# Anima-Lab/MaskDiT

Measured on AMD Instinct MI355X. Metric: training img/sec MaskDiT-XL/2 256 mask=0.5 bs=1024, higher is better.
Workload: dtype bf16; 1 GPU; DiT-XL/2 ImageNet256-latent [32x32x4], mask_ratio=0.5, mae_loss_coef=0.1, sample(moments)+class-dropout+fwd+bwd+grad-allreduce+AdamW+EMA, random-init (de-zeroed) weights; global_batch=1024, per_gpu_batch=1024, micro_batch=1024, accum=1, parallelism=dp1

## Files before the change

maskdit_amd/csrc/attention.hip:

```cpp
#include "common.h"
#include <type_traits>
#include "../../include/maskdit_hip.h"

template <int HD>
struct AttnCfg {
  static constexpr int HDK = (HD + 31) / 32 * 32;
  static constexpr int HDN = (HD + 15) / 16 * 16;
  static constexpr int KSTEPS = HDK / 32;
  static constexpr int NFRAG = HDN / 16;
  static constexpr int CH = HD / 8;
  static constexpr int PITCH_CH = (HDK / 8) | 1;
  static constexpr int PITCH = PITCH_CH * 16;
  static constexpr int TILE_BYTES = 64 * PITCH;
};

template <int HD> struct AttnRow {
  static constexpr int NFRAG = AttnCfg<HD>::NFRAG;
  static constexpr int NP = (NFRAG / 2 < HD / 32) ? NFRAG / 2 : HD / 32;
  static constexpr int NT = NFRAG - 2 * NP;
  uint4 pr[NP > 0 ? NP : 1];
  uint2 tl[NT > 0 ? NT : 1];
};
__device__ __forceinline__ unsigned attn_pack2(float a, float b) {
  bf16x2 t;
// ... 666 lines not shown
    for (int qi = 0; qi < QF; ++qi) {
#pragma unroll
      for (int f = 0; f < C::NFRAG; ++f) o[qi][f] = (f32x4){0.f, 0.f, 0.f, 0.f};
      m_run[qi] = -1e30f;
      l_run[qi] = 0.f;
    }
#pragma unroll 1
    for (int kb = 0; kb < L; kb += KB) {
      f32x4 s[QF][KB / 16];
#pragma unroll
      for (int f = 0; f < KB / 16; ++f) {
#pragma unroll
        for (int qi = 0; qi < QF; ++qi) s[qi][f] = (f32x4){0.f, 0.f, 0.f, 0.f};
#pragma unroll
        for (int ks = 0; ks < C::KSTEPS; ++ks) {
          const bf16x8 kfr = sp_frag_rows<HD, L>(Ks, kb + 16 * f + i16, ks, g);
#pragma unroll
          for (int qi = 0; qi < QF; ++qi) s[qi][f] = mfma16(kfr, qf[qi][ks], s[qi][f]);
        }
      }
      bf16x8 pf[QF][KB / 32];
      if (kb + KB > Lv) {
#pragma unroll
        for (int qi = 0; qi < QF; ++qi)
#pragma unroll
          for (int f = 0; f < KB / 16; ++f)
#pragma unroll
            for (int r = 0; r < 4; ++r) s[qi][f][r] = (kb + 16 * f + 4 * g + r < Lv) ? s[qi][f][r] : -1e30f;
      }
#pragma unroll
      for (int qi = 0; qi < QF; ++qi) {
        float mx = -1e30f;
#pragma unroll
        for (int f = 0; f < KB / 16; ++f)
#pragma unroll
          for (int r = 0; r < 4; ++r) mx = fmaxf(mx, s[qi][f][r]);
        mx = group_max(mx);
        const float m_new = fmaxf(m_run[qi], mx * scale_log2e);
        const float alpha = fast_exp2(m_run[qi] - m_new);
        float psum = 0.f;
#pragma unroll
        for (int f = 0; f < KB / 16; ++f)
#pragma unroll
          for (int r = 0; r < 4; ++r) {
            const float pv = fast_exp2(__builtin_fmaf(s[qi][f][r], scale_log2e, -m_new));
            s[qi][f][r] = pv;
            psum += pv;
          }
        l_run[qi] = l_run[qi] * alpha + psum;
        m_run[qi] = m_new;
#pragma unroll
        for (int f = 0; f < C::NFRAG; ++f)
#pragma unroll
          for (int r = 0; r < 4; ++r) o[qi][f][r] *= alpha;
#pragma unroll
        for (int ks = 0; ks < KB / 32; ++ks) pf[qi][ks] = pack_pair(s[qi][2 * ks], s[qi][2 * ks + 1]);
      }
#pragma unroll
      for (int ks = 0; ks < KB / 32; ++ks)
#pragma unroll
        for (int f = 0; f < C::NFRAG; ++f) {
          const bf16x8 vfr = sp_frag_cols<HD, L>(Vs, kb + 32 * ks, f, i16, g);
#pragma unroll
          for (int qi = 0; qi < QF; ++qi) o[qi][f] = mfma16(vfr, pf[qi][ks], o[qi][f]);
        }
    }
#pragma unroll
    for (int qi = 0; qi < QF; ++qi) {
      const int q = wave * 16 * KF + 16 * (qp + qi) + i16;
      const float l_tot = group_sum(l_run[qi]);
      const float inv = 1.f / l_tot;
      bf16* orow = out + ((long)b * L + q) * D + h * HD;
      AttnRow<HD> orw;
      attn_pack_row<HD>(orw, o[qi], inv);
      attn_store_row<HD>(orow, g, orw);
      if (g == 0) lse[((long)b * H + h) * L + q] = m_run[qi] + log2f(l_tot);
    }
  }
}

__device__ __forceinline__ void sp_item_coords(int item, int B, int H, int& b, int& h) {
  const int full = (B >> 3) << 3;
  int sid;
  if (item < full * H) {
    const int xcd = item & 7, k = item >> 3;
    const int grp = k / H;
    sid = (grp * 8 + xcd) * H + (k - grp * H);
  } else {
    sid = item;
  }
  b = sid / H;
  h = sid - b * H;
}

#define SP_LDS_BARRIER()                                 \
  {                                                      \
    asm volatile("s_waitcnt lgkmcnt(0)" ::: "memory");   \
    __builtin_amdgcn_s_barrier();                        \
    asm volatile("" ::: "memory");                       \
  }
template <int HD, int KF, int OCC>
__global__ __launch_bounds__(512, OCC) void attn_bwd_sp_kernel(const bf16* __restrict__ qkv, const bf16* __restrict__ out,
                                                              const bf16* __restrict__ dout, const float* __restrict__ lse,
                                                              float* __restrict__ delta, bf16* __restrict__ dqkv, int H,
                                                              float scale, float scale_log2e, int Lv, int B, int dbg) {
  using C = SpCfg<HD>;
  constexpr int L = 128 * KF;
  constexpr int TILE = L * C::PITCH;
  __shared__ __attribute__((aligned(16))) char smem[4 * TILE + 2 * L * 4 + 64];
  char* Qs = smem;
  char* Ks = smem + TILE;
  char* Vs = smem + 2 * TILE;
  char* dOs = smem + 3 * TILE;
  float* lse_s = (float*)(smem + 4 * TILE);
  float* del_s = lse_s + L;
  const int tid = threadIdx.x, lane = tid & 63, wave = tid >> 6;
  const int i16 = lane & 15, g = lane >> 4;
  const int D = H * HD;
  const long ld = 3L * D;
  const int nitems = B * H;

  SpRegs<HD, L> r0, r1, r2, r3;
  bf16x8 of[KF][C::KSTEPS], dof[KF][C::KSTEPS];
  float lse_r = 0.f;
  auto fetch = [&](int item) {
    int b, h;
    sp_item_coords(item, B, H, b, h);
    const bf16* base = qkv + (long)b * L * ld + h * HD;
    const bf16* dobase = dout + (long)b * L * D + h * HD;
    const bf16* obase = out + (long)b * L * D + h * HD;
    sp_load_nb<HD, L>(r0, base, ld, tid);
    sp_load_nb<HD, L>(r1, base + D, ld, tid);
    sp_load_nb<HD, L>(r2, base + 2 * D, ld, tid);
    sp_load_nb<HD, L>(r3, dobase, D, tid);
    lse_r = lse[((long)b * H + h) * L + (tid & (L - 1))];
#pragma unroll
    for (int qi = 0; qi < KF; ++qi) {
      const int q = wave * 16 * KF + 16 * qi + i16;
#pragma unroll
      for (int s = 0; s < C::KSTEPS; ++s) {
        const int d = min(32 * s + 8 * g, HD - 8);
        of[qi][s] = *(const bf16x8*)(obase + (long)q * D + d);
        dof[qi][s] = *(const bf16x8*)(dobase + (long)q * D + d);
      }
    }
  };

  auto stage = [&](int it) {
    int b, h;
    sp_item_coords(it, B, H, b, h);
    const long bh = (long)b * H + h;
    sp_store<HD, L>(r0, Qs, tid);
    sp_store<HD, L>(r1, Ks, tid);
    sp_store<HD, L>(r2, Vs, tid);
    sp_store<HD, L>(r3, dOs, tid);
    if (tid < L) lse_s[tid] = lse_r;
#pragma unroll
    for (int qi = 0; qi < KF; ++qi) {
      const int q = wave * 16 * KF + 16 * qi + i16;
      float dl = 0.f;
#pragma unroll
      for (int s = 0; s < C::KSTEPS; ++s) {
        float part = 0.f;
#pragma unroll
        for (int e = 0; e < 8; ++e) part += bf2f(dof[qi][s][e]) * bf2f(of[qi][s][e]);
        dl += (32 * s + 8 * g < HD) ? part : 0.f;
      }
      dl = group_sum(dl);
      if (g == 0) {
        del_s[q] = dl * scale;
        delta[bh * L + q] = dl;
      }
    }
  };

  int item = blockIdx.x;
  if (item >= nitems) return;
  fetch(item);
  stage(item);
  for (;;) {
    int b, h;
    sp_item_coords(item, B, H, b, h);
    SP_LDS_BARRIER()
    const bool has_next = OCC == 2 && item + (int)gridDim.x < nitems;
    if (has_next && !MDT_EXP(dbg & 2)) fetch(item + gridDim.x);
    __builtin_amdgcn_sched_barrier(0);

#pragma unroll 1
    for (int ki = 0; ki < (MDT_EXP(dbg & 4) ? 0 : KF); ++ki) {
      const int k0 = wave * 16 * KF + 16 * ki;
      bf16x8 kf[C::KSTEPS], vf[C::KSTEPS];
#pragma unroll
      for (int ks = 0; ks < C::KSTEPS; ++ks) {
        kf[ks] = sp_frag_rows<HD, L>(Ks, k0 + i16, ks, g);
        vf[ks] = sp_frag_rows<HD, L>(Vs, k0 + i16, ks, g);
      }
      f32x4 dk[C::NFRAG], dv[C::NFRAG];
#pragma unroll
      for (int f = 0; f < C::NFRAG; ++f) {
        dk[f] = (f32x4){0.f, 0.f, 0.f, 0.f};
        dv[f] = (f32x4){0.f, 0.f, 0.f, 0.f};
      }
      const bool key_ok = (k0 + i16) < Lv;
#pragma unroll 1
      for (int qb = 0; qb < L; qb += 64) {
        f32x4 pm[4], ds[4];
#pragma unroll
        for (int f = 0; f < 4; ++f) {
          f32x4 s = (f32x4){0.f, 0.f, 0.f, 0.f}, dp = (f32x4){0.f, 0.f, 0.f, 0.f};
#pragma unroll
          for (int ks = 0; ks < C::KSTEPS; ++ks) {
            s = mfma16(sp_frag_rows<HD, L>(Qs, qb + 16 * f + i16, ks, g), kf[ks], s);
            dp = mfma16(sp_frag_rows<HD, L>(dOs, qb + 16 * f + i16, ks, g), vf[ks], dp);
          }
          const f32x4 ls = *(const f32x4*)(lse_s + qb + 16 * f + 4 * g);
          const f32x4 dl = *(const f32x4*)(del_s + qb + 16 * f + 4 * g);
#pragma unroll
          for (int r = 0; r < 4; ++r) {
            const float pv = fast_exp2(__builtin_fmaf(s[r], scale_log2e, -ls[r]));
            pm[f][r] = pv;
            ds[f][r] = pv * __builtin_fmaf(dp[r], scale, -dl[r]);
          }
        }
#pragma unroll
        for (int ks = 0; ks < 2; ++ks) {
          const bf16x8 pf = pack_pair(pm[2 * ks], pm[2 * ks + 1]);
          const bf16x8 dsf = pack_pair(ds[2 * ks], ds[2 * ks + 1]);
#pragma unroll
          for (int f = 0; f < C::NFRAG; ++f) {
            dv[f] = mfma16(sp_frag_cols<HD, L>(dOs, qb + 32 * ks, f, i16, g), pf, dv[f]);
            dk[f] = mfma16(sp_frag_cols<HD, L>(Qs, qb + 32 * ks, f, i16, g), dsf, dk[f]);
          }
        }
      }
      bf16* drow = dqkv + ((long)b * L + k0 + i16) * ld + h * HD;
      AttnRow<HD> krw, vrw;
      if (!key_ok) {
#pragma unroll
        for (int f = 0; f < C::NFRAG; ++f) dk[f] = dv[f] = (f32x4){0.f, 0.f, 0.f, 0.f};
      }
      attn_pack_row<HD>(krw, dk);
      attn_pack_row<HD>(vrw, dv);
      if (!MDT_EXP(dbg & 1)) {
        attn_store_row<HD>(drow + D, g, krw);
        attn_store_row<HD>(drow + 2 * D, g, vrw);
      }
    }

#pragma unroll 1
    for (int qi = 0; qi < (MDT_EXP(dbg & 8) ? 0 : KF); ++qi) {
      const int q = wave * 16 * KF + 16 * qi + i16;
      bf16x8 qf[C::KSTEPS], dqo[C::KSTEPS];
#pragma unroll
      for (int ks = 0; ks < C::KSTEPS; ++ks) {
        qf[ks] = sp_frag_rows<HD, L>(Qs, q, ks, g);
        dqo[ks] = sp_frag_rows<HD, L>(dOs, q, ks, g);
      }
      const float my_lse = lse_s[q], dl = del_s[q];
      f32x4 dq[C::NFRAG];
#pragma unroll
      for (int f = 0; f < C::NFRAG; ++f) dq[f] = (f32x4){0.f, 0.f, 0.f, 0.f};
#pragma unroll 1
      for (int kb = 0; kb < L; kb += 64) {
        f32x4 ds[4];
#pragma unroll
        for (int f = 0; f < 4; ++f) {
          f32x4 s = (f32x4){0.f, 0.f, 0.f, 0.f}, dp = (f32x4){0.f, 0.f, 0.f, 0.f};
#pragma unroll
          for (int ks = 0; ks < C::KSTEPS; ++ks) {
            s = mfma16(sp_frag_rows<HD, L>(Ks, kb + 16 * f + i16, ks, g), qf[ks], s);
            dp = mfma16(sp_frag_rows<HD, L>(Vs, kb + 16 * f + i16, ks, g), dqo[ks], dp);
          }
#pragma unroll
          for (int r = 0; r < 4; ++r) {
            const float pv = fast_exp2(__builtin_fmaf(s[r], scale_log2e, -my_lse));
            ds[f][r] = pv * __builtin_fmaf(dp[r], scale, -dl);
          }
        }
        if (kb + 64 > Lv) {
#pragma unroll
          for (int f = 0; f < 4; ++f)
#pragma unroll
            for (int r = 0; r < 4; ++r) ds[f][r] = (kb + 16 * f + 4 * g + r < Lv) ? ds[f][r] : 0.f;
        }
#pragma unroll
        for (int ks = 0; ks < 2; ++ks) {
          const bf16x8 dsf = pack_pair(ds[2 * ks], ds[2 * ks + 1]);
#pragma unroll
          for (int f = 0; f < C::NFRAG; ++f) dq[f] = mfma16(sp_frag_cols<HD, L>(Ks, kb + 32 * ks, f, i16, g), dsf, dq[f]);
        }
      }
      bf16* drow = dqkv + ((long)b * L + q) * ld + h * HD;
      AttnRow<HD> qrw;
      attn_pack_row<HD>(qrw, dq);
      if (!MDT_EXP(dbg & 1)) attn_store_row<HD>(drow, g, qrw);
    }
    if (!has_next) break;
    SP_LDS_BARRIER()
    item += gridDim.x;
    stage(item);
  }
}

template <int HD>
__device__ __forceinline__ void attn_bwd_item_math(const char* Qs, const char* Ks, const char* Vs, const char* dOs,
                                                   const float* lse_s, const float* del_s, bf16* dbase, long ld, int D,
                                                   int wave, int i16, int g, int Lv, float scale, float scale_log2e,
                                                   AttnRow<HD>& q_cur, const AttnRow<HD>& q_prev) {
  using C = SpCfg<HD>;
  constexpr int L = 128;
  AttnRow<HD> k_keep, v_keep;
  {
    const int k0 = wave * 16;
    bf16x8 kf[C::KSTEPS], vf[C::KSTEPS];
#pragma unroll
    for (int ks = 0; ks < C::KSTEPS; ++ks) {
      kf[ks] = sp_frag_rows<HD, L>(Ks, k0 + i16, ks, g);
      vf[ks] = sp_frag_rows<HD, L>(Vs, k0 + i16, ks, g);
    }
    f32x4 dk[C::NFRAG], dv[C::NFRAG];
#pragma unroll
    for (int f = 0; f < C::NFRAG; ++f) {
      dk[f] = (f32x4){0.f, 0.f, 0.f, 0.f};
      dv[f] = (f32x4){0.f, 0.f, 0.f, 0.f};
    }
    const bool key_ok = (k0 + i16) < Lv;
#pragma unroll 1
    for (int qb = 0; qb < L; qb += 64) {
      f32x4 pm[4], ds[4];
#pragma unroll
      for (int f = 0; f < 4; ++f) {
        f32x4 s = (f32x4){0.f, 0.f, 0.f, 0.f}, dp = (f32x4){0.f, 0.f, 0.f, 0.f};
#pragma unroll
        for (int ks = 0; ks < C::KSTEPS; ++ks) {
          s = mfma16(sp_frag_rows<HD, L>(Qs, qb + 16 * f + i16, ks, g), kf[ks], s);
          dp = mfma16(sp_frag_rows<HD, L>(dOs, qb + 16 * f + i16, ks, g), vf[ks], dp);
        }
        const f32x4 ls = *(const f32x4*)(lse_s + qb + 16 * f + 4 * g);
        const f32x4 dl = *(const f32x4*)(del_s + qb + 16 * f + 4 * g);
#pragma unroll
        for (int r = 0; r < 4; ++r) {
          const float pv = fast_exp2(__builtin_fmaf(s[r], scale_log2e, -ls[r]));
          pm[f][r] = pv;
          ds[f][r] = pv * __builtin_fmaf(dp[r], scale, -dl[r]);
        }
      }
#pragma unroll
      for (int ks = 0; ks < 2; ++ks) {
        const bf16x8 pf = pack_pair(pm[2 * ks], pm[2 * ks + 1]);
        const bf16x8 dsf = pack_pair(ds[2 * ks], ds[2 * ks + 1]);
#pragma unroll
        for (int f = 0; f < C::NFRAG; ++f) {
          dv[f] = mfma16(sp_frag_cols<HD, L>(dOs, qb + 32 * ks, f, i16, g), pf, dv[f]);
          dk[f] = mfma16(sp_frag_cols<HD, L>(Qs, qb + 32 * ks, f, i16, g), dsf, dk[f]);
        }
      }
    }
    bf16* drow = dbase + (long)(k0 + i16) * ld;
    if (!key_ok) {
#pragma unroll
      for (int f = 0; f < C::NFRAG; ++f) dk[f] = dv[f] = (f32x4){0.f, 0.f, 0.f, 0.f};
    }
    attn_pack_row<HD>(k_keep, dk);
    attn_pack_row<HD>(v_keep, dv);
    attn_store_row<HD>(drow + D, g, k_keep);
    attn_store_row<HD>(drow + 2 * D, g, v_keep);
    attn_keep_alive<HD>(q_prev);
  }
  {
    const int q = wave * 16 + i16;
    bf16x8 qf[C::KSTEPS], dqo[C::KSTEPS];
#pragma unroll
    for (int ks = 0; ks < C::KSTEPS; ++ks) {
      qf[ks] = sp_frag_rows<HD, L>(Qs, q, ks, g);
      dqo[ks] = sp_frag_rows<HD, L>(dOs, q, ks, g);
    }
    const float my_lse = lse_s[q], dl = del_s[q];
    f32x4 dq[C::NFRAG];
#pragma unroll
    for (int f = 0; f < C::NFRAG; ++f) dq[f] = (f32x4){0.f, 0.f, 0.f, 0.f};
#pragma unroll 1
    for (int kb = 0; kb < L; kb += 64) {
      f32x4 ds[4];
#pragma unroll
      for (int f = 0; f < 4; ++f) {
        f32x4 s = (f32x4){0.f, 0.f, 0.f, 0.f}, dp = (f32x4){0.f, 0.f, 0.f, 0.f};
#pragma unroll
        for (int ks = 0; ks < C::KSTEPS; ++ks) {
          s = mfma16(sp_frag_rows<HD, L>(Ks, kb + 16 * f + i16, ks, g), qf[ks], s);
          dp = mfma16(sp_frag_rows<HD, L>(Vs, kb + 16 * f + i16, ks, g), dqo[ks], dp);
        }
#pragma unroll
        for (int r = 0; r < 4; ++r) {
          const float pv = fast_exp2(__builtin_fmaf(s[r], scale_log2e, -my_lse));
          ds[f][r] = pv * __builtin_fmaf(dp[r], scale, -dl);
        }
      }
      if (kb + 64 > Lv) {
#pragma unroll
        for (int f = 0; f < 4; ++f)
#pragma unroll
          for (int r = 0; r < 4; ++r) ds[f][r] = (kb + 16 * f + 4 * g + r < Lv) ? ds[f][r] : 0.f;
      }
#pragma unroll
      for (int ks = 0; ks < 2; ++ks) {
        const bf16x8 dsf = pack_pair(ds[2 * ks], ds[2 * ks + 1]);
#pragma unroll
        for (int f = 0; f < C::NFRAG; ++f) dq[f] = mfma16(sp_frag_cols<HD, L>(Ks, kb + 32 * ks, f, i16, g), dsf, dq[f]);
      }
    }
    bf16* drow = dbase + (long)q * ld;
    attn_pack_row<HD>(q_cur, dq);
    attn_store_row<HD>(drow, g, q_cur);
    attn_keep_alive<HD>(k_keep);
    attn_keep_alive<HD>(v_keep);
  }
}

template <int HD>
__global__ __launch_bounds__(512, 2) void attn_bwd_dma_kernel(const bf16* __restrict__ qkv, const bf16* __restrict__ out,
                                                               const bf16* __restrict__ dout, const float* __restrict__ lse,
                                                               float* __restrict__ delta, bf16* __restrict__ dqkv, int H,
                                                               float scale, float scale_log2e, int Lv, int B) {
  using C = SpCfg<HD>;
  static_assert(C::PITCH == HD * 2, "tile rows must be contiguous in LDS (odd chunk count)");
  constexpr int L = 128;
  constexpr int TILE = L * C::PITCH;
  constexpr int HALF_CH = L * C::CH / 2;
  static_assert(HALF_CH % 64 == 0, "a wave moves whole 1-KiB pieces");
  constexpr int NDMA = HALF_CH / 64;
  constexpr int NSTORE = 1 + 3 * (AttnRow<HD>::NP + AttnRow<HD>::NT);
  __shared__ __attribute__((aligned(16))) char buf0[4 * TILE];
  __shared__ __attribute__((aligned(16))) char buf1[4 * TILE];
  __shared__ float lse_s0[L], lse_s1[L], del_s[L];
  const int tid = threadIdx.x, lane = tid & 63;
  const int wave = __builtin_amdgcn_readfirstlane(tid >> 6);
  const int i16 = lane & 15, g = lane >> 4;
  const int D = H * HD;
  const long ld = 3L * D;
  const int nitems = B * H;

  static_assert(NDMA == 9, "nine 1-KiB pieces per wave");
  const int tw = wave >> 1, hw = wave & 1;
  const long row_bytes = (tw < 3 ? ld : (long)D) * 2;
  unsigned doff[NDMA];
  int lds_main, lds_tail;
  if constexpr (sp_split<HD, L>) {
#pragma unroll
    for (int j = 0; j < 8; ++j) {
      const int r = 64 * hw + 8 * j + (lane >> 3), c = (lane & 7) ^ (lane >> 3);
      doff[j] = (unsigned)(r * row_bytes + c * 16);
    }
    doff[8] = (unsigned)((64 * hw + lane) * row_bytes + 128);
    lds_main = tw * TILE + hw * 8192;
    lds_tail = tw * TILE + L * 128 + hw * 1024;
  } else {
#pragma unroll
    for (int j = 0; j < NDMA; ++j) {
      const int idx = hw * HALF_CH + 64 * j + lane;
      const int r = idx / C::CH, c = idx - r * C::CH;
      doff[j] = (unsigned)(r * row_bytes + c * 16);
    }
    lds_main = tw * TILE + hw * HALF_CH * 16;
    lds_tail = lds_main + 8192;
  }
  auto item_src = [&](int item) -> const char* {
    int b, h;
    sp_item_coords(item, B, H, b, h);
    return tw < 3 ? (const char*)(qkv + (long)b * L * ld + h * HD + tw * D) : (const char*)(dout + (long)b * L * D + h * HD);
  };

  float lse_r = 0.f;
  bf16x8 of0[C::KSTEPS], of1[C::KSTEPS];
  AttnRow<HD> qk0, qk1;
#pragma unroll
  for (int q = 0; q < (AttnRow<HD>::NP > 0 ? AttnRow<HD>::NP : 1); ++q) qk0.pr[q] = qk1.pr[q] = make_uint4(0u, 0u, 0u, 0u);
#pragma unroll
  for (int t = 0; t < (AttnRow<HD>::NT > 0 ? AttnRow<HD>::NT : 1); ++t) qk0.tl[t] = qk1.tl[t] = make_uint2(0u, 0u);
  const int qrow = wave * 16 + i16;

#define ATTN_DMA_BARRIER()                                                                    \
  {                                                                                           \
    asm volatile("s_waitcnt lgkmcnt(0)" ::: "memory");                                        \
    __builtin_amdgcn_s_barrier();                                                             \
    asm volatile("" ::: "memory");                                                            \
  }
#define ATTN_DMA_BODY(P, CUR, NXT, LSE_CUR, LSE_NXT, OF_CUR, OF_NXT, QK_CUR, QK_PRV, VMWAIT)                             \
  {                                                                                                        \
    int b, h;                                                                                              \
    sp_item_coords(item, B, H, b, h);                                                                      \
    const long bh = (long)b * H + h;                                                                       \
    const char* Qs = CUR;                                                                                  \
    const char* Ks = CUR + TILE;                                                                           \
    const char* Vs = CUR + 2 * TILE;                                                                       \
    const char* dOs = CUR + 3 * TILE;                                                                      \
                                                                        \
    asm volatile("; MDT_CHK hand_wait" ::: "memory");                                                      \
    __builtin_amdgcn_s_waitcnt(((VMWAIT) & 15) | (7 << 4) | (15 << 8) | (((VMWAIT) >> 4) << 14));  \
    asm volatile("" ::: "memory");                                                                         \
    if (tid < L) LSE_CUR[tid] = lse_r;                                                                     \
    asm volatile("; MDT_CHK no_dma" ::: "memory");  \
    ATTN_DMA_BARRIER()                \
    const int nxt = item + (int)gridDim.x;                                                                 \
    {       \
      const int fit = nxt < nitems ? nxt : item;                                                           \
      const char* src = item_src(fit);                                                                     \
      _Pragma("unroll") for (int j = 0; j < 8; ++j) glds16(src + opaque(doff[j]), NXT + lds_main + 1024 * j); \
      glds16(src + opaque(doff[8]), NXT + lds_tail);                                                       \
      int nb, nh;                                                                                          \
      sp_item_coords(fit, B, H, nb, nh);                                                                   \
      lse_r = lse[((long)nb * H + nh) * L + (tid & (L - 1))];                                              \
      const bf16* orow = out + ((long)nb * L + qrow) * D + nh * HD;                                        \
      _Pragma("unroll") for (int s2 = 0; s2 < C::KSTEPS; ++s2)                                             \
        OF_NXT[s2] = *(const bf16x8*)(orow + min(32 * s2 + 8 * g, HD - 8));                                \
    }                                                                                                      \
    __builtin_amdgcn_sched_barrier(0);                                                                     \
    {                                                   \
      float dl = 0.f;                                                                                      \
      _Pragma("unroll") for (int s2 = 0; s2 < C::KSTEPS; ++s2) {                                           \
        const bf16x8 dof = sp_frag_rows<HD, L>(dOs, qrow, s2, g);                                             \
        float part = 0.f;                                                                                  \
        _Pragma("unroll") for (int e = 0; e < 8; ++e) part += bf2f(dof[e]) * bf2f(OF_CUR[s2][e]);          \
        dl += (32 * s2 + 8 * g < HD) ? part : 0.f;                                                         \
      }                                                                                                    \
      dl = group_sum(dl);                                                                                  \
      if (g == 0) {                                                                                        \
        del_s[qrow] = dl * scale;              \
        delta[bh * L + qrow] = dl;                                                                         \
      }                                                                                                    \
    }                                                                                                      \
    ATTN_DMA_BARRIER()                                               \
    attn_bwd_item_math<HD>(Qs, Ks, Vs, dOs, LSE_CUR, del_s, dqkv + (long)b * L * ld + h * HD, ld, D, wave, i16, g, Lv, \
                           scale, scale_log2e, QK_CUR, QK_PRV);                                            \
    item = nxt;                                                                                            \
  }

  int item = blockIdx.x;
  if (item >= nitems) return;
  {
    const char* src = item_src(item);
#pragma unroll
    for (int j = 0; j < 8; ++j) glds16(src + opaque(doff[j]), buf0 + lds_main + 1024 * j);
    glds16(src + opaque(doff[8]), buf0 + lds_tail);
    int b, h;
    sp_item_coords(item, B, H, b, h);
    lse_r = lse[((long)b * H + h) * L + (tid & (L - 1))];
    const bf16* orow = out + ((long)b * L + qrow) * D + h * HD;
#pragma unroll
    for (int s2 = 0; s2 < C::KSTEPS; ++s2) of0[s2] = *(const bf16x8*)(orow + min(32 * s2 + 8 * g, HD - 8));
#pragma unroll
    for (int s2 = 0; s2 < C::KSTEPS; ++s2) of1[s2] = of0[s2];
  }
#ifdef MDT_REGRESS_R3_ATTN_WAIT
  ATTN_DMA_BODY(0, buf0, buf1, lse_s0, lse_s1, of0, of1, qk0, qk1, NSTORE)
#else
  ATTN_DMA_BODY(0, buf0, buf1, lse_s0, lse_s1, of0, of1, qk0, qk1, 0)
#endif
  while (item < nitems) {
    ATTN_DMA_BODY(1, buf1, buf0, lse_s1, lse_s0, of1, of0, qk1, qk0, NSTORE)
    if (item >= nitems) break;
    ATTN_DMA_BODY(0, buf0, buf1, lse_s0, lse_s1, of0, of1, qk0, qk1, NSTORE)
  }
#undef ATTN_DMA_BODY
#undef ATTN_DMA_BARRIER
}

template <int HD, int KF>
__global__ __launch_bounds__(512, 2) void attn_bwd_q_res_kernel(const bf16* __restrict__ qkv, const bf16* __restrict__ out,
                                                                 const bf16* __restrict__ dout, const float* __restrict__ lse,
                                                                 float* __restrict__ delta, bf16* __restrict__ dqkv, int H,
                                                                 float scale, float scale_log2e, int Lv) {
  using C = SpCfg<HD>;
  constexpr int L = 128 * KF;
  constexpr int TILE = L * sp_pitch<HD, L>;
  __shared__ __attribute__((aligned(16))) char smem[2 * TILE + 64];
  char* Ks = smem;
  char* Vs = smem + TILE;
  const int tid = threadIdx.x, lane = tid & 63, wave = tid >> 6;
  const int i16 = lane & 15, g = lane >> 4;
  int b, h;
  sp_block_coords(gridDim.y / H, H, b, h);
  const long bh = (long)b * H + h;
  const int D = H * HD;
  const long ld = 3L * D;
  const bf16* base = qkv + (long)b * L * ld + h * HD;
  {
    SpRegs<HD, L> kreg, vreg;
    sp_load_nb<HD, L>(kreg, base + D, ld, tid);
    sp_load_nb<HD, L>(vreg, base + 2 * D, ld, tid);
    sp_store<HD, L>(kreg, Ks, tid);
    sp_store<HD, L>(vreg, Vs, tid);
  }
  __syncthreads();
#pragma unroll 1
  for (int qi = 0; qi < KF; ++qi) {
    const int q = wave * 16 * KF + 16 * qi + i16;
    const long orow = ((long)b * L + q) * D + h * HD;
    bf16x8 qf[C::KSTEPS], dqo[C::KSTEPS], of[C::KSTEPS];
#pragma unroll
    for (int s2 = 0; s2 < C::KSTEPS; ++s2) {
      const int d = min(32 * s2 + 8 * g, HD - 8);
      qf[s2] = *(const bf16x8*)(base + (long)q * ld + d);
      dqo[s2] = *(const bf16x8*)(dout + orow + d);
      of[s2] = *(const bf16x8*)(out + orow + d);
    }
    const float my_lse = lse[bh * L + q];
    float dl = 0.f;
#pragma unroll
    for (int s2 = 0; s2 < C::KSTEPS; ++s2) {
      const bool in = 32 * s2 + 8 * g < HD;
      float part = 0.f;
#pragma unroll
      for (int e = 0; e < 8; ++e) {
        part += bf2f(dqo[s2][e]) * bf2f(of[s2][e]);
        qf[s2][e] = in ? qf[s2][e] : (bf16)0.f;
        dqo[s2][e] = in ? dqo[s2][e] : (bf16)0.f;
      }
      dl += in ? part : 0.f;
    }
    dl = group_sum(dl);
    if (g == 0) delta[bh * L + q] = dl;
    const float dl_s = dl * scale;
    f32x4 dq[C::NFRAG];
#pragma unroll
    for (int f = 0; f < C::NFRAG; ++f) dq[f] = (f32x4){0.f, 0.f, 0.f, 0.f};
#pragma unroll 1
    for (int kb = 0; kb < L; kb += 64) {
      f32x4 ds[4];
#pragma unroll
      for (int f = 0; f < 4; ++f) {
        f32x4 sv = (f32x4){0.f, 0.f, 0.f, 0.f}, dp = (f32x4){0.f, 0.f, 0.f, 0.f};
#pragma unroll
        for (int ks = 0; ks < C::KSTEPS; ++ks) {
          sv = mfma16(sp_frag_rows<HD, L>(Ks, kb + 16 * f + i16, ks, g), qf[ks], sv);
          dp = mfma16(sp_frag_rows<HD, L>(Vs, kb + 16 * f + i16, ks, g), dqo[ks], dp);
        }
#pragma unroll
        for (int r = 0; r < 4; ++r) {
          const float pv = fast_exp2(__builtin_fmaf(sv[r], scale_log2e, -my_lse));
          ds[f][r] = pv * __builtin_fmaf(dp[r], scale, -dl_s);
        }
      }
      if (kb + 64 > Lv) {
#pragma unroll
        for (int f = 0; f < 4; ++f)
#pragma unroll
          for (int r = 0; r < 4; ++r) ds[f][r] = (kb + 16 * f + 4 * g + r < Lv) ? ds[f][r] : 0.f;
      }
#pragma unroll
      for (int ks = 0; ks < 2; ++ks) {
        const bf16x8 dsf = pack_pair(ds[2 * ks], ds[2 * ks + 1]);
#pragma unroll
        for (int f = 0; f < C::NFRAG; ++f) dq[f] = mfma16(sp_frag_cols<HD, L>(Ks, kb + 32 * ks, f, i16, g), dsf, dq[f]);
      }
    }
    bf16* drow = dqkv + ((long)b * L + q) * ld + h * HD;
    AttnRow<HD> qrw;
    attn_pack_row<HD>(qrw, dq);
    attn_store_row<HD>(drow, g, qrw);
  }
}

template <int HD, int KF>
__global__ __launch_bounds__(512, 2) void attn_bwd_kv_res_kernel(const bf16* __restrict__ qkv, const bf16* __restrict__ dout,
                                                                  const float* __restrict__ lse, const float* __restrict__ delta,
                                                                  bf16* __restrict__ dqkv, int H, float scale,
                                                                  float scale_log2e, int Lv) {
  using C = SpCfg<HD>;
  constexpr int L = 128 * KF;
  constexpr int TILE = L * sp_pitch<HD, L>;
  __shared__ __attribute__((aligned(16))) char smem[2 * TILE + 2 * L * 4 + 64];
  char* Qs = smem;
  char* dOs = smem + TILE;
  float* lse_s = (float*)(smem + 2 * TILE);
  float* del_s = lse_s + L;
  const int tid = threadIdx.x, lane = tid & 63, wave = tid >> 6;
  const int i16 = lane & 15, g = lane >> 4;
  int b, h;
  sp_block_coords(gridDim.y / H, H, b, h);
  const long bh = (long)b * H + h;
  const int D = H * HD;
  const long ld = 3L * D;
  const bf16* base = qkv + (long)b * L * ld + h * HD;
  {
    SpRegs<HD, L> qreg, doreg;
    sp_load_nb<HD, L>(qreg, base, ld, tid);
    sp_load_nb<HD, L>(doreg, dout + (long)b * L * D + h * HD, D, tid);
    float ls[(L + 511) / 512], dd[(L + 511) / 512];
#pragma unroll
    for (int k = 0; k < (L + 511) / 512; ++k) {
      ls[k] = lse[bh * L + ((tid + 512 * k) & (L - 1))];
      dd[k] = delta[bh * L + ((tid + 512 * k) & (L - 1))];
    }
    sp_store<HD, L>(qreg, Qs, tid);
    sp_store<HD, L>(doreg, dOs, tid);
#pragma unroll
    for (int k = 0; k < (L + 511) / 512; ++k)
      if (tid + 512 * k < L) {
        lse_s[tid + 512 * k] = ls[k];
        del_s[tid + 512 * k] = dd[k] * scale;
      }
  }
  __syncthreads();
#pragma unroll 1
  for (int ki = 0; ki < KF; ++ki) {
    const int k0 = wave * 16 * KF + 16 * ki;
    bf16x8 kf[C::KSTEPS], vf[C::KSTEPS];
#pragma unroll
    for (int s2 = 0; s2 < C::KSTEPS; ++s2) {
      const int d = min(32 * s2 + 8 * g, HD - 8);
      kf[s2] = *(const bf16x8*)(base + (long)(k0 + i16) * ld + D + d);
      vf[s2] = *(const bf16x8*)(base + (long)(k0 + i16) * ld + 2 * D + d);
    }
#pragma unroll
    for (int s2 = 0; s2 < C::KSTEPS; ++s2) {
      const bool in = 32 * s2 + 8 * g < HD;
#pragma unroll
      for (int e = 0; e < 8; ++e) {
        kf[s2][e] = in ? kf[s2][e] : (bf16)0.f;
        vf[s2][e] = in ? vf[s2][e] : (bf16)0.f;
      }
    }
    f32x4 dk[C::NFRAG], dv[C::NFRAG];
#pragma unroll
    for (int f = 0; f < C::NFRAG; ++f) {
      dk[f] = (f32x4){0.f, 0.f, 0.f, 0.f};
      dv[f] = (f32x4){0.f, 0.f, 0.f, 0.f};
    }
    const float key_pen = (k0 + i16) < Lv ? 0.f : 1e30f;
#pragma unroll 1
    for (int qb = 0; qb < L; qb += 64) {
      f32x4 pm[4], ds[4];
#pragma unroll
      for (int f = 0; f < 4; ++f) {
        f32x4 sv = (f32x4){0.f, 0.f, 0.f, 0.f}, dp = (f32x4){0.f, 0.f, 0.f, 0.f};
#pragma unroll
        for (int ks = 0; ks < C::KSTEPS; ++ks) {
          sv = mfma16(sp_frag_rows<HD, L>(Qs, qb + 16 * f + i16, ks, g), kf[ks], sv);
          dp = mfma16(sp_frag_rows<HD, L>(dOs, qb + 16 * f + i16, ks, g), vf[ks], dp);
        }
        const f32x4 ls = *(const f32x4*)(lse_s + qb + 16 * f + 4 * g);
        const f32x4 dl = *(const f32x4*)(del_s + qb + 16 * f + 4 * g);
#pragma unroll
        for (int r = 0; r < 4; ++r) {
          const float pv = fast_exp2(__builtin_fmaf(sv[r], scale_log2e, -ls[r]) - key_pen);
          pm[f][r] = pv;
          ds[f][r] = pv * __builtin_fmaf(dp[r], scale, -dl[r]);
        }
      }
#pragma unroll
      for (int ks = 0; ks < 2; ++ks) {
        const bf16x8 pf = pack_pair(pm[2 * ks], pm[2 * ks + 1]);
        const bf16x8 dsf = pack_pair(ds[2 * ks], ds[2 * ks + 1]);
#pragma unroll
        for (int f = 0; f < C::NFRAG; ++f) {
          dv[f] = mfma16(sp_frag_cols<HD, L>(dOs, qb + 32 * ks, f, i16, g), pf, dv[f]);
          dk[f] = mfma16(sp_frag_cols<HD, L>(Qs, qb + 32 * ks, f, i16, g), dsf, dk[f]);
        }
      }
    }
    bf16* drow = dqkv + ((long)b * L + k0 + i16) * ld + h * HD;
    AttnRow<HD> krw, vrw;
    if (key_pen != 0.f) {
#pragma unroll
      for (int f = 0; f < C::NFRAG; ++f) dk[f] = dv[f] = (f32x4){0.f, 0.f, 0.f, 0.f};
    }
    attn_pack_row<HD>(krw, dk);
    attn_pack_row<HD>(vrw, dv);
    attn_store_row<HD>(drow + D, g, krw);
    attn_store_row<HD>(drow + 2 * D, g, vrw);
  }
}


#define ATTN_DISPATCH(HD_, CALL) \
  switch (HD_) {                 \
    case 32: { constexpr int HDc = 32; CALL; } break; \
    case 64: { constexpr int HDc = 64; CALL; } break; \
    case 72: { constexpr int HDc = 72; CALL; } break; \
    case 80: { constexpr int HDc = 80; CALL; } break; \
    default: mdt_set_error("attention: head_dim must be one of 32, 64, 72, 80"); return MDT_ERR_ARG; \
  }

int nt8_num_cus();
static int attn_num_cus() { return nt8_num_cus() & ~7; }

extern "C" int mdt_attn_fwd(const mdt_bf16* qkv, mdt_bf16* out, float* lse, int B, int L, int H, int hd, int L_valid,
                            mdt_stream_t stream) {
  MDT_REQUIRE(qkv && out && lse, "attn_fwd: null pointer");
  MDT_REQUIRE(B > 0 && H > 0 && L > 0 && L % 64 == 0, "attn_fwd: L must be a positive multiple of 64");
  if (L_valid <= 0 || L_valid > L) L_valid = L;
  float sl = (1.0f / sqrtf((float)hd)) * 1.4426950408889634f;
  if ((L == 128 || L == 256) && mdt_get_tuning_int(MDT_TUNE_ATTN_SP) != 1) {
    dim3 grid(1, B * H);
    const bool pad = L_valid < L;
    if (L == 128 && !pad) {
      ATTN_DISPATCH(hd, hipLaunchKernelGGL((attn_fwd_sp_kernel<HDc, 1, false>), grid, dim3(512), 0, (hipStream_t)stream,
                                           (const bf16*)qkv, (bf16*)out, lse, H, sl, L_valid));
    } else if (L == 128) {
      ATTN_DISPATCH(hd, hipLaunchKernelGGL((attn_fwd_sp_kernel<HDc, 1, true>), grid, dim3(512), 0, (hipStream_t)stream,
                                           (const bf16*)qkv, (bf16*)out, lse, H, sl, L_valid));
    } else if (!pad) {
      ATTN_DISPATCH(hd, hipLaunchKernelGGL((attn_fwd_sp_kernel<HDc, 2, false>), grid, dim3(512), 0, (hipStream_t)stream,
                                           (const bf16*)qkv, (bf16*)out, lse, H, sl, L_valid));
    } else {
      ATTN_DISPATCH(hd, hipLaunchKernelGGL((attn_fwd_sp_kernel<HDc, 2, true>), grid, dim3(512), 0, (hipStream_t)stream,
                                           (const bf16*)qkv, (bf16*)out, lse, H, sl, L_valid));
    }
    return mdt_check_launch("attn_fwd_sp");
  }
  if (L == 512 && hd == 72 && mdt_get_tuning_int(MDT_TUNE_ATTN_SP) != 1) {
    if (L_valid < L)
      hipLaunchKernelGGL((attn_fwd_sp_kernel<72, 4, true>), dim3(1, B * H), dim3(512), 0, (hipStream_t)stream, (const bf16*)qkv,
                         (bf16*)out, lse, H, sl, L_valid);
    else
      hipLaunchKernelGGL((attn_fwd_sp_kernel<72, 4, false>), dim3(1, B * H), dim3(512), 0, (hipStream_t)stream, (const bf16*)qkv,
                         (bf16*)out, lse, H, sl, L_valid);
    return mdt_check_launch("attn_fwd_sp");
  }
  if (L == 1024 && hd == 32 && mdt_get_tuning_int(MDT_TUNE_ATTN_SP) != 1) {
    hipLaunchKernelGGL((attn_fwd_res_kernel<32, 8>), dim3(1, B * H), dim3(512), 0, (hipStream_t)stream, (const bf16*)qkv,
                       (bf16*)out, lse, H, sl, L_valid);
    return mdt_check_launch("attn_fwd_res");
  }
  const int qf_knob = mdt_get_tuning_int(MDT_TUNE_ATTN_QF);
  if (L % 128 == 0 && (qf_knob == 2 || (qf_knob == 0 && hd <= 64))) {
    dim3 grid(L / 128, B * H);
    ATTN_DISPATCH(hd, hipLaunchKernelGGL((attn_fwd_kernel<HDc, 2>), grid, dim3(256), 0, (hipStream_t)stream,
                                         (const bf16*)qkv, (bf16*)out, lse, L, H, sl, L_valid));
  } else {
    dim3 grid(L / 64, B * H);
    ATTN_DISPATCH(hd, hipLaunchKernelGGL((attn_fwd_kernel<HDc, 1>), grid, dim3(256), 0, (hipStream_t)stream,
                                         (const bf16*)qkv, (bf16*)out, lse, L, H, sl, L_valid));
  }
  return mdt_check_launch("attn_fwd");
}

extern "C" int mdt_attn_bwd(const mdt_bf16* qkv, const mdt_bf16* out, const mdt_bf16* dout, const float* lse,
                            float* delta, mdt_bf16* dqkv, int B, int L, int H, int hd, int L_valid,
                            mdt_stream_t stream) {
  MDT_REQUIRE(qkv && out && dout && lse && delta && dqkv, "attn_bwd: null pointer");
  MDT_REQUIRE(B > 0 && H > 0 && L > 0 && L % 64 == 0, "attn_bwd: L must be a positive multiple of 64");
  if (L_valid <= 0 || L_valid > L) L_valid = L;
  float sc = 1.0f / sqrtf((float)hd);
  float sl = sc * 1.4426950408889634f;
  const int sp_knob = mdt_get_tuning_int(MDT_TUNE_ATTN_SP);
  const int adbg = MDT_EXP(1) ? mdt_get_tuning_int(MDT_TUNE_ATTN_DBG) : 0;
  const bool sp_ok = L == 128 || (L == 256 && (hd == 32 || hd == 64 || hd == 72));
  if (sp_ok && sp_knob != 1 && (L == 128 || hd <= 64 || sp_knob == 2)) {
    dim3 g1(B * H);
    const int items = B * H;
    const int cus = attn_num_cus();
    dim3 gp(items < cus ? items : cus);
    if (L == 128 && hd == 72 && sp_knob != 2 && sp_knob != 3) {
      hipLaunchKernelGGL(attn_bwd_dma_kernel<72>, gp, dim3(512), 0, (hipStream_t)stream, (const bf16*)qkv, (const bf16*)out,
                         (const bf16*)dout, lse, delta, (bf16*)dqkv, H, sc, sl, L_valid, B);
    } else if (L == 128 && sp_knob == 2) {
      ATTN_DISPATCH(hd, hipLaunchKernelGGL((attn_bwd_sp_kernel<HDc, 1, 4>), g1, dim3(512), 0, (hipStream_t)stream,
                                           (const bf16*)qkv, (const bf16*)out, (const bf16*)dout, lse, delta, (bf16*)dqkv, H,
                                           sc, sl, L_valid, B, adbg));
    } else if (L == 128) {
      ATTN_DISPATCH(hd, hipLaunchKernelGGL((attn_bwd_sp_kernel<HDc, 1, 2>), gp, dim3(512), 0, (hipStream_t)stream,
                                           (const bf16*)qkv, (const bf16*)out, (const bf16*)dout, lse, delta, (bf16*)dqkv, H,
                                           sc, sl, L_valid, B, adbg));
    } else {
      switch (hd) {
        case 32: hipLaunchKernelGGL((attn_bwd_sp_kernel<32, 2, 2>), gp, dim3(512), 0, (hipStream_t)stream, (const bf16*)qkv,
                                    (const bf16*)out, (const bf16*)dout, lse, delta, (bf16*)dqkv, H, sc, sl, L_valid, B, adbg); break;
        case 64: hipLaunchKernelGGL((attn_bwd_sp_kernel<64, 2, 2>), gp, dim3(512), 0, (hipStream_t)stream, (const bf16*)qkv,
                                    (const bf16*)out, (const bf16*)dout, lse, delta, (bf16*)dqkv, H, sc, sl, L_valid, B, adbg); break;
        default: hipLaunchKernelGGL((attn_bwd_sp_kernel<72, 2, 2>), gp, dim3(512), 0, (hipStream_t)stream, (const bf16*)qkv,
                                    (const bf16*)out, (const bf16*)dout, lse, delta, (bf16*)dqkv, H, sc, sl, L_valid, B, adbg); break;
      }
    }
    return mdt_check_launch("attn_bwd_sp");
  }
  if (L == 512 && hd == 72 && sp_knob != 1) {
    hipLaunchKernelGGL((attn_bwd_q_res_kernel<72, 4>), dim3(1, B * H), dim3(512), 0, (hipStream_t)stream, (const bf16*)qkv,
                       (const bf16*)out, (const bf16*)dout, lse, delta, (bf16*)dqkv, H, sc, sl, L_valid);
    int rc = mdt_check_launch("attn_bwd_q_res");
    if (rc) return rc;
    hipLaunchKernelGGL((attn_bwd_kv_res_kernel<72, 4>), dim3(1, B * H), dim3(512), 0, (hipStream_t)stream, (const bf16*)qkv,
                       (const bf16*)dout, lse, delta, (bf16*)dqkv, H, sc, sl, L_valid);
    return mdt_check_launch("attn_bwd_kv_res");
  }
  if (L == 1024 && hd == 32 && sp_knob != 1) {
    hipLaunchKernelGGL((attn_bwd_q_res_kernel<32, 8>), dim3(1, B * H), dim3(512), 0, (hipStream_t)stream, (const bf16*)qkv,
                       (const bf16*)out, (const bf16*)dout, lse, delta, (bf16*)dqkv, H, sc, sl, L_valid);
    int rc = mdt_check_launch("attn_bwd_q_res");
    if (rc) return rc;
    hipLaunchKernelGGL((attn_bwd_kv_res_kernel<32, 8>), dim3(1, B * H), dim3(512), 0, (hipStream_t)stream, (const bf16*)qkv,
                       (const bf16*)dout, lse, delta, (bf16*)dqkv, H, sc, sl, L_valid);
    return mdt_check_launch("attn_bwd_kv_res");
  }
  dim3 grid(L / 64, B * H);
  ATTN_DISPATCH(hd, hipLaunchKernelGGL(attn_bwd_dq_kernel<HDc>, grid, dim3(256), 0, (hipStream_t)stream,
                                       (const bf16*)qkv, (const bf16*)out, (const bf16*)dout, lse, delta,
                                       (bf16*)dqkv, L, H, sc, sl, L_valid));
  int rc = mdt_check_launch("attn_bwd_dq");
  if (rc) return rc;
  ATTN_DISPATCH(hd, hipLaunchKernelGGL(attn_bwd_dkv_kernel<HDc>, grid, dim3(256), 0, (hipStream_t)stream,
                                       (const bf16*)qkv, (const bf16*)dout, lse, delta, (bf16*)dqkv, L, H, sc, sl, L_valid));
  return mdt_check_launch("attn_bwd_dkv");
}
```

Baseline: 2263 img/s.

## Reuse dS from the dK/dV pass for dQ via an LDS transpose

The default DMA attention backward kernel (hd=72, L=128) now stores the bf16 dS fragments computed during the dK/dV phase into an LDS image that overlays the V/dO tiles. The dQ phase then reads them back with transposed LDS reads, so it no longer recomputes QK^T, dO·V^T and the exponentials. This removes roughly half of the backward MFMA and exp work in exchange for extra LDS writes, two barriers, and more register pressure from holding dS. The old two-phase recompute path stays available behind tuning knob 4.

```diff
diff --git a/maskdit_amd/csrc/attention.hip b/maskdit_amd/csrc/attention.hip
--- a/maskdit_amd/csrc/attention.hip
+++ b/maskdit_amd/csrc/attention.hip
@@ -992,14 +992,16 @@
   }
 }
 
-template <int HD>
+constexpr int ATTN_DS_PITCH = 128 * 2 + 16;
+template <int HD, bool SS>
 __device__ __forceinline__ void attn_bwd_item_math(const char* Qs, const char* Ks, const char* Vs, const char* dOs,
                                                    const float* lse_s, const float* del_s, bf16* dbase, long ld, int D,
                                                    int wave, int i16, int g, int Lv, float scale, float scale_log2e,
-                                                   AttnRow<HD>& q_cur, const AttnRow<HD>& q_prev) {
+                                                   AttnRow<HD>& q_cur, const AttnRow<HD>& q_prev, char* dS_img) {
   using C = SpCfg<HD>;
   constexpr int L = 128;
   AttnRow<HD> k_keep, v_keep;
+  bf16x8 ds_keep[SS ? 2 : 1][2];
   {
     const int k0 = wave * 16;
     bf16x8 kf[C::KSTEPS], vf[C::KSTEPS];
@@ -1015,7 +1017,8 @@
       dv[f] = (f32x4){0.f, 0.f, 0.f, 0.f};
     }
     const bool key_ok = (k0 + i16) < Lv;
-#pragma unroll 1
+    constexpr int QB_UNROLL = SS ? 2 : 1;
+#pragma unroll QB_UNROLL
     for (int qb = 0; qb < L; qb += 64) {
       f32x4 pm[4], ds[4];
 #pragma unroll
@@ -1044,6 +1047,7 @@
           dv[f] = mfma16(sp_frag_cols<HD, L>(dOs, qb + 32 * ks, f, i16, g), pf, dv[f]);
           dk[f] = mfma16(sp_frag_cols<HD, L>(Qs, qb + 32 * ks, f, i16, g), dsf, dk[f]);
         }
+        if constexpr (SS) ds_keep[qb >> 6][ks] = dsf;
       }
     }
     bf16* drow = dbase + (long)(k0 + i16) * ld;
@@ -1056,62 +1060,97 @@
     attn_store_row<HD>(drow + D, g, k_keep);
     attn_store_row<HD>(drow + 2 * D, g, v_keep);
     attn_keep_alive<HD>(q_prev);
-  }
-  {
+    if constexpr (SS) {
+      if (k0 + 16 > Lv) {
+        bf16x8 z;
+#pragma unroll
+        for (int e = 0; e < 8; ++e) z[e] = (bf16)0.f;
+#pragma unroll
+        for (int j = 0; j < 4; ++j) ds_keep[j >> 1][j & 1] = key_ok ? ds_keep[j >> 1][j & 1] : z;
+      }
+      SP_LDS_BARRIER()
+      char* row = dS_img + (k0 + i16) * ATTN_DS_PITCH + 8 * g;
+#pragma unroll
+      for (int j = 0; j < 4; ++j) {
+        const uint4 v = __builtin_bit_cast(uint4, ds_keep[j >> 1][j & 1]);
+        *(uint2*)(row + 64 * j) = make_uint2(v.x, v.y);
+        *(uint2*)(row + 64 * j + 32) = make_uint2(v.z, v.w);
+      }
+      SP_LDS_BARRIER()
+    }
+  }
+  if constexpr (SS) {
     const int q = wave * 16 + i16;
-    bf16x8 qf[C::KSTEPS], dqo[C::KSTEPS];
-#pragma unroll
-    for (int ks = 0; ks < C::KSTEPS; ++ks) {
-      qf[ks] = sp_frag_rows<HD, L>(Qs, q, ks, g);
-      dqo[ks] = sp_frag_rows<HD, L>(dOs, q, ks, g);
-    }
-    const float my_lse = lse_s[q], dl = del_s[q];
     f32x4 dq[C::NFRAG];
 #pragma unroll
     for (int f = 0; f < C::NFRAG; ++f) dq[f] = (f32x4){0.f, 0.f, 0.f, 0.f};
-#pragma unroll 1
-    for (int kb = 0; kb < L; kb += 64) {
-      f32x4 ds[4];
-#pragma unroll
-      for (int f = 0; f < 4; ++f) {
-        f32x4 s = (f32x4){0.f, 0.f, 0.f, 0.f}, dp = (f32x4){0.f, 0.f, 0.f, 0.f};
-#pragma unroll
-        for (int ks = 0; ks < C::KSTEPS; ++ks) {
-          s = mfma16(sp_frag_rows<HD, L>(Ks, kb + 16 * f + i16, ks, g), qf[ks], s);
-          dp = mfma16(sp_frag_rows<HD, L>(Vs, kb + 16 * f + i16, ks, g), dqo[ks], dp);
-        }
-#pragma unroll
-        for (int r = 0; r < 4; ++r) {
-          const float pv = fast_exp2(__builtin_fmaf(s[r], scale_log2e, -my_lse));
-          ds[f][r] = pv * __builtin_fmaf(dp[r], scale, -dl);
-        }
-      }
-      if (kb + 64 > Lv) {
-#pragma unroll
-        for (int f = 0; f < 4; ++f)
-#pragma unroll
-          for (int r = 0; r < 4; ++r) ds[f][r] = (kb + 16 * f + 4 * g + r < Lv) ? ds[f][r] : 0.f;
-      }
-#pragma unroll
-      for (int ks = 0; ks < 2; ++ks) {
-        const bf16x8 dsf = pack_pair(ds[2 * ks], ds[2 * ks + 1]);
-#pragma unroll
-        for (int f = 0; f < C::NFRAG; ++f) dq[f] = mfma16(sp_frag_cols<HD, L>(Ks, kb + 32 * ks, f, i16, g), dsf, dq[f]);
-      }
+#pragma unroll
+    for (int kb = 0; kb < L; kb += 32) {
+      const char* p = dS_img + (kb + 4 * g + (i16 >> 2)) * ATTN_DS_PITCH + (16 * wave + 4 * (i16 & 3)) * 2;
+      const bf16x8 dsf = cat4(lds_tr_read(p), lds_tr_read(p + 16 * ATTN_DS_PITCH));
+#pragma unroll
+      for (int f = 0; f < C::NFRAG; ++f) dq[f] = mfma16(sp_frag_cols<HD, L>(Ks, kb, f, i16, g), dsf, dq[f]);
     }
     bf16* drow = dbase + (long)q * ld;
     attn_pack_row<HD>(q_cur, dq);
     attn_store_row<HD>(drow, g, q_cur);
     attn_keep_alive<HD>(k_keep);
     attn_keep_alive<HD>(v_keep);
-  }
-}
-
-template <int HD>
-__global__ __launch_bounds__(512, 2) void attn_bwd_dma_kernel(const bf16* __restrict__ qkv, const bf16* __restrict__ out,
-                                                               const bf16* __restrict__ dout, const float* __restrict__ lse,
-                                                               float* __restrict__ delta, bf16* __restrict__ dqkv, int H,
-                                                               float scale, float scale_log2e, int Lv, int B) {
+  } else {
+    const int q = wave * 16 + i16;
+    bf16x8 qf[C::KSTEPS], dqo[C::KSTEPS];
+#pragma unroll
+    for (int ks = 0; ks < C::KSTEPS; ++ks) {
+      qf[ks] = sp_frag_rows<HD, L>(Qs, q, ks, g);
+      dqo[ks] = sp_frag_rows<HD, L>(dOs, q, ks, g);
+    }
+    const float my_lse = lse_s[q], dl = del_s[q];
+    f32x4 dq[C::NFRAG];
+#pragma unroll
+    for (int f = 0; f < C::NFRAG; ++f) dq[f] = (f32x4){0.f, 0.f, 0.f, 0.f};
+#pragma unroll 1
+    for (int kb = 0; kb < L; kb += 64) {
+      f32x4 ds[4];
+#pragma unroll
+      for (int f = 0; f < 4; ++f) {
+        f32x4 s = (f32x4){0.f, 0.f, 0.f, 0.f}, dp = (f32x4){0.f, 0.f, 0.f, 0.f};
+#pragma unroll
+        for (int ks = 0; ks < C::KSTEPS; ++ks) {
+          s = mfma16(sp_frag_rows<HD, L>(Ks, kb + 16 * f + i16, ks, g), qf[ks], s);
+          dp = mfma16(sp_frag_rows<HD, L>(Vs, kb + 16 * f + i16, ks, g), dqo[ks], dp);
+        }
+#pragma unroll
+        for (int r = 0; r < 4; ++r) {
+          const float pv = fast_exp2(__builtin_fmaf(s[r], scale_log2e, -my_lse));
+          ds[f][r] = pv * __builtin_fmaf(dp[r], scale, -dl);
+        }
+      }
+      if (kb + 64 > Lv) {
+#pragma unroll
+        for (int f = 0; f < 4; ++f)
+#pragma unroll
+          for (int r = 0; r < 4; ++r) ds[f][r] = (kb + 16 * f + 4 * g + r < Lv) ? ds[f][r] : 0.f;
+      }
+#pragma unroll
+      for (int ks = 0; ks < 2; ++ks) {
+        const bf16x8 dsf = pack_pair(ds[2 * ks], ds[2 * ks + 1]);
+#pragma unroll
+        for (int f = 0; f < C::NFRAG; ++f) dq[f] = mfma16(sp_frag_cols<HD, L>(Ks, kb + 32 * ks, f, i16, g), dsf, dq[f]);
+      }
+    }
+    bf16* drow = dbase + (long)q * ld;
+    attn_pack_row<HD>(q_cur, dq);
+    attn_store_row<HD>(drow, g, q_cur);
+    attn_keep_alive<HD>(k_keep);
+    attn_keep_alive<HD>(v_keep);
+  }
+}
+
+template <int HD, bool SS>
+__device__ __forceinline__ void attn_bwd_dma_body(const bf16* __restrict__ qkv, const bf16* __restrict__ out,
+                                                  const bf16* __restrict__ dout, const float* __restrict__ lse,
+                                                  float* __restrict__ delta, bf16* __restrict__ dqkv, int H,
+                                                  float scale, float scale_log2e, int Lv, int B) {
   using C = SpCfg<HD>;
   static_assert(C::PITCH == HD * 2, "tile rows must be contiguous in LDS (odd chunk count)");
   constexpr int L = 128;
@@ -1131,6 +1170,7 @@
   const int nitems = B * H;
 
   static_assert(NDMA == 9, "nine 1-KiB pieces per wave");
+  static_assert(!SS || L * ATTN_DS_PITCH <= 2 * TILE, "the dS image overlays the V and dO tiles");
   const int tw = wave >> 1, hw = wave & 1;
   const long row_bytes = (tw < 3 ? ld : (long)D) * 2;
   unsigned doff[NDMA];
@@ -1220,8 +1260,8 @@
       }                                                                                                    \
     }                                                                                                      \
     ATTN_DMA_BARRIER()                                               \
-    attn_bwd_item_math<HD>(Qs, Ks, Vs, dOs, LSE_CUR, del_s, dqkv + (long)b * L * ld + h * HD, ld, D, wave, i16, g, Lv, \
-                           scale, scale_log2e, QK_CUR, QK_PRV);                                            \
+    attn_bwd_item_math<HD, SS>(Qs, Ks, Vs, dOs, LSE_CUR, del_s, dqkv + (long)b * L * ld + h * HD, ld, D, wave, i16, g, \
+                               Lv, scale, scale_log2e, QK_CUR, QK_PRV, CUR + 2 * TILE);                    \
     item = nxt;                                                                                            \
   }
 
@@ -1242,7 +1282,7 @@
     for (int s2 = 0; s2 < C::KSTEPS; ++s2) of1[s2] = of0[s2];
   }
 #ifdef MDT_REGRESS_R3_ATTN_WAIT
-  ATTN_DMA_BODY(0, buf0, buf1, lse_s0, lse_s1, of0, of1, qk0, qk1, NSTORE)
+  ATTN_DMA_BODY(0, buf0, buf1, lse_s0, lse_s1, of0, of1, qk0, qk1, (SS ? NSTORE : 0))
 #else
   ATTN_DMA_BODY(0, buf0, buf1, lse_s0, lse_s1, of0, of1, qk0, qk1, 0)
 #endif
@@ -1253,6 +1293,20 @@
   }
 #undef ATTN_DMA_BODY
 #undef ATTN_DMA_BARRIER
+}
+template <int HD>
+__global__ __launch_bounds__(512, 2) void attn_bwd_dma_kernel(const bf16* __restrict__ qkv, const bf16* __restrict__ out,
+                                                               const bf16* __restrict__ dout, const float* __restrict__ lse,
+                                                               float* __restrict__ delta, bf16* __restrict__ dqkv, int H,
+                                                               float scale, float scale_log2e, int Lv, int B) {
+  attn_bwd_dma_body<HD, true>(qkv, out, dout, lse, delta, dqkv, H, scale, scale_log2e, Lv, B);
+}
+template <int HD>
+__global__ __launch_bounds__(512, 2) void attn_bwd_dma_twophase_kernel(const bf16* __restrict__ qkv, const bf16* __restrict__ out,
+                                                                        const bf16* __restrict__ dout, const float* __restrict__ lse,
+                                                                        float* __restrict__ delta, bf16* __restrict__ dqkv, int H,
+                                                                        float scale, float scale_log2e, int Lv, int B) {
+  attn_bwd_dma_body<HD, false>(qkv, out, dout, lse, delta, dqkv, H, scale, scale_log2e, Lv, B);
 }
 
 template <int HD, int KF>
@@ -1543,8 +1597,12 @@
     const int cus = attn_num_cus();
     dim3 gp(items < cus ? items : cus);
     if (L == 128 && hd == 72 && sp_knob != 2 && sp_knob != 3) {
-      hipLaunchKernelGGL(attn_bwd_dma_kernel<72>, gp, dim3(512), 0, (hipStream_t)stream, (const bf16*)qkv, (const bf16*)out,
-                         (const bf16*)dout, lse, delta, (bf16*)dqkv, H, sc, sl, L_valid, B);
+      if (sp_knob == 4)
+        hipLaunchKernelGGL(attn_bwd_dma_twophase_kernel<72>, gp, dim3(512), 0, (hipStream_t)stream, (const bf16*)qkv,
+                           (const bf16*)out, (const bf16*)dout, lse, delta, (bf16*)dqkv, H, sc, sl, L_valid, B);
+      else
+        hipLaunchKernelGGL(attn_bwd_dma_kernel<72>, gp, dim3(512), 0, (hipStream_t)stream, (const bf16*)qkv,
+                           (const bf16*)out, (const bf16*)dout, lse, delta, (bf16*)dqkv, H, sc, sl, L_valid, B);
     } else if (L == 128 && sp_knob == 2) {
       ATTN_DISPATCH(hd, hipLaunchKernelGGL((attn_bwd_sp_kernel<HDc, 1, 4>), g1, dim3(512), 0, (hipStream_t)stream,
                                            (const bf16*)qkv, (const bf16*)out, (const bf16*)dout, lse, delta, (bf16*)dqkv, H,
```

Result: no change. 2277 img/s (median of 6 runs) (+0.6%).
